# liruiw/OMG-Planner

Measured on AMD Instinct MI355X. Metric: CHOMP iterations/sec (batched scenes) + ms/plan, Panda 7-DoF 30-wp, higher is better.
Workload: dtype f32 SDF / f64 kinematics+update; 1 GPU; 100 table-top scenes/GPU x (64-goal goal-set cost + CHOMP step), Panda 9-dof, 30 waypoints; scenes_per_gpu=100, total_scenes=100, goals=64, waypoints=30, sdf_grid=4x64^3 + 128x96x32 per scene, private, goal_selection=MD on device (omgx_goal_update_optimize), pipeline_parts=3, top_k_collision=1000, plan_restart_every_steps=50

## Files before the change

### omg-planner_amd/csrc/omg_device.h

```cpp
#pragma once
#include <hip/hip_runtime.h>
#include <stdint.h>

#include "../../include/omg_hip.h"

#define OMG_WAVE 64

namespace omg {

struct __attribute__((packed, aligned(4))) F2 { float a, b; };
struct __attribute__((packed, aligned(4))) F4 { float a, b, c, d; };

__device__ __forceinline__ float lerpf(float a, float b, float t) { return __builtin_fmaf(t, b - a, a); }

struct Axis { int i0; float f; bool ok; };
__device__ __forceinline__ Axis axis_of(float g) {
    Axis a;
    a.ok = (g > -1.0e9f) && (g <= 1.0e9f);
    const float s = g - 0.5f;
    a.i0 = (int)s;
    a.f = s - (float)a.i0;
    const bool edge = (s == -1.0f) && (g > -0.5f);
    a.i0 = edge ? 0 : a.i0;
    a.f = edge ? -1.0f : a.f;
// ... 165 lines not shown
        fmx = sdf_value(G, axm, ay, az);
        fmy = sdf_value(G, ax, aym, az);
        fmz = sdf_value(G, ax, ay, azm);
    }
    const float g0 = (float)(0.5 * (double)(fpx - fmx) * o.rdelta);
    const float g1 = (float)(0.5 * (double)(fpy - fmy) * o.rdelta);
    const float g2 = (float)(0.5 * (double)(fpz - fmz) * o.rdelta);
    float v0, v1, v2;
    if (value <= 0.0f) {
        acc.pot += (float)(-(double)value + 0.5 * (double)o.eps);
        v0 = -g0; v1 = -g1; v2 = -g2;
    } else {
        const float d = value - o.eps;
        acc.pot += o.i2eps * d * d * o.pad;
        const float ie = o.ieps;
        v0 = ie * g0 * d * o.pad; v1 = ie * g1 * d * o.pad; v2 = ie * g2 * d * o.pad;
    }
    acc.gx += __builtin_fmaf(T[8], v2, __builtin_fmaf(T[4], v1, T[0] * v0));
    acc.gy += __builtin_fmaf(T[9], v2, __builtin_fmaf(T[5], v1, T[1] * v0));
    acc.gz += __builtin_fmaf(T[10], v2, __builtin_fmaf(T[6], v1, T[2] * v0));
}

template <bool WANT_GRAD>
__device__ __forceinline__ void sdf_pair(const ObjParams& o, const float* __restrict__ grid, float px, float py, float pz,
                                         Accum& acc) {
    const PairPrep pp = pair_prepare(o, px, py, pz);
    if (!pp.far) pair_exact<WANT_GRAD>(o, grid, pp.tx, pp.ty, pp.tz, acc);
}

#define OMG_CONST_AS __attribute__((address_space(4)))
typedef const OMG_CONST_AS omgx_object* ObjTablePtr;
typedef const OMG_CONST_AS int32_t* IntTablePtr;
#define OMG_GLOBAL_AS __attribute__((address_space(1)))
typedef const OMG_GLOBAL_AS char* GlobalBytes;
typedef float F2v __attribute__((ext_vector_type(2), aligned(4)));
__device__ __forceinline__ F2 global_f2(GlobalBytes p) { const F2v v = *(const OMG_GLOBAL_AS F2v*)p; return F2{v.x, v.y}; }
__device__ __forceinline__ ObjTablePtr as_const(const omgx_object* p) { return (ObjTablePtr)(uintptr_t)p; }
__device__ __forceinline__ IntTablePtr as_const(const int32_t* p) { return (IntTablePtr)(uintptr_t)p; }

__device__ __forceinline__ ObjParams load_object(ObjTablePtr ob) {
    ObjParams o;
#pragma unroll
    for (int k = 0; k < 12; ++k) o.T[k] = ob->pose_inv[k];
#pragma unroll
    for (int k = 0; k < 3; ++k) { o.lo[k] = ob->lo[k]; o.hi[k] = ob->hi[k]; o.dim[k] = ob->dim[k]; }
    o.delta = ob->delta; o.eps = ob->epsilon; o.pad = ob->padding_scale; o.clr = ob->clearance;
#pragma unroll
    for (int k = 0; k < 3; ++k) { o.rw[k] = ob->inv_extent[k]; o.rc[k] = ob->rb_c[k]; o.rh[k] = ob->rb_h[k]; }
    o.rr2 = ob->rb_r2;
    o.rdelta = ob->inv_delta; o.i2eps = ob->inv_2eps; o.ieps = ob->inv_eps;
    return o;
}

template <bool WANT_GRAD>
__device__ __forceinline__ Accum sdf_point(const omgx_object* __restrict__ objs, int o_begin, int o_end,
                                           const float* __restrict__ pool, float px, float py, float pz) {
    Accum acc{0.0f, 0.0f, 0.0f, 0.0f, 0.0f};
    for (int o = o_begin; o < o_end; ++o) {
        ObjTablePtr ob = as_const(objs) + o;
        if (ob->disabled > 0) continue;
        const ObjParams op = load_object(ob);
        sdf_pair<WANT_GRAD>(op, pool + ob->grid_offset, px, py, pz, acc);
    }
    return acc;
}

__device__ __forceinline__ void gq_warm_scalar_cache(const omgx_object* objects, int o_begin, int o_end, const double* balls) {
    const omgx_object* ob[8];
#pragma unroll
    for (int k = 0; k < 8; ++k) ob[k] = objects + (o_begin + k < o_end ? o_begin + k : o_end - 1);
#define OMG_WARM_OBJ(N) "s_load_dword s96, %" #N ", 0x0\n\ts_load_dword s97, %" #N ", 0x40\n\ts_load_dword s98, %" #N ", 0x80\n\ts_load_dword s99, %" #N ", 0xb4\n\t"
    asm volatile(OMG_WARM_OBJ(0) OMG_WARM_OBJ(1) OMG_WARM_OBJ(2) OMG_WARM_OBJ(3) OMG_WARM_OBJ(4) OMG_WARM_OBJ(5) OMG_WARM_OBJ(6) OMG_WARM_OBJ(7)
                 "s_load_dword s96, %8, 0x0\n\ts_load_dword s97, %8, 0x40\n\ts_load_dword s98, %8, 0x80\n\ts_load_dword s99, %8, 0xc0\n\t"
                 "s_load_dword s96, %8, 0x100\n\ts_load_dword s97, %8, 0x13c\n\ts_waitcnt lgkmcnt(0)"
                 :
                 : "s"(ob[0]), "s"(ob[1]), "s"(ob[2]), "s"(ob[3]), "s"(ob[4]), "s"(ob[5]), "s"(ob[6]), "s"(ob[7]), "s"(balls)
                 : "s96", "s97", "s98", "s99", "memory");
#undef OMG_WARM_OBJ
}

template <class DPtr>
struct RobotViewT {
    const double* __restrict__ raw;
    DPtr d;
    const double* __restrict__ g;
    int P;
    __device__ __forceinline__ RobotViewT(const double* blob, int P_) : raw(blob), d((DPtr)(uintptr_t)(blob + OMGX_ROBOT_POINTS + 30 * P_)), g(blob + OMGX_ROBOT_POINTS + 30 * P_), P(P_) {}
    __device__ __forceinline__ RobotViewT(const double* blob, int P_, DPtr chain_constants) : raw(blob), d(chain_constants), g(blob + OMGX_ROBOT_POINTS + 30 * P_), P(P_) {}
    __device__ __forceinline__ DPtr uvw(int i) const { return d + 27 * i; }
    __device__ __forceinline__ DPtr tp(int i) const { return d + 189 + 3 * i; }
    __device__ __forceinline__ DPtr hand() const { return d + 210; }
    __device__ __forceinline__ DPtr lf() const { return d + 222; }
    __device__ __forceinline__ DPtr rf() const { return d + 234; }
    __device__ __forceinline__ const double* pts(int l, int p) const { return g + 246 + 3 * (l * P + p); }
    __device__ __forceinline__ DPtr ax(int l) const { return d + 246 + 30 * P + 3 * l; }
    __device__ __forceinline__ DPtr og(int l) const { return d + 276 + 30 * P + 3 * l; }
    __device__ __forceinline__ double radius(int l) const { return d[306 + 30 * P + l]; }
    __device__ __forceinline__ DPtr ball(int l) const { return d + 316 + 30 * P + 4 * l; }
    __device__ __forceinline__ const double* lower() const { return raw + OMGX_ROBOT_LOWER; }
    __device__ __forceinline__ const double* upper() const { return raw + OMGX_ROBOT_UPPER; }
};
typedef RobotViewT<const double*> RobotView;
typedef RobotViewT<const OMG_CONST_AS double*> RobotViewS;

struct Pose { double R[9]; double t[3]; };

// ... 229 lines not shown
```

### omg-planner_amd/csrc/omg_goalset_queue.h

```cpp
#pragma once

#define GQ_TBL_MAX 32
#ifndef GQ_WG_PER_CU
#define GQ_WG_PER_CU 5
#endif
#ifndef GQ_WAVES
#define GQ_WAVES 4
#endif
#define GQ_NT (64 * GQ_WAVES)

struct GqFar {
    float T[12], lo[3], rc[3], rh[3], rr2, rb_r;
    bool cullable;
    int disabled;
};

typedef uint32_t GqU16 __attribute__((ext_vector_type(16)));
typedef uint32_t GqU8 __attribute__((ext_vector_type(8)));
typedef uint32_t GqU4 __attribute__((ext_vector_type(4)));
static_assert(offsetof(omgx_object, pose_inv) == 0 && offsetof(omgx_object, lo) == 0x30 && offsetof(omgx_object, epsilon) == 0x58 &&
              offsetof(omgx_object, clearance) == 0x60 && offsetof(omgx_object, disabled) == 0x64 && offsetof(omgx_object, rb_c) == 0x88 &&
              offsetof(omgx_object, rb_h) == 0x94 && offsetof(omgx_object, rb_r) == 0xa0 && offsetof(omgx_object, rb_r2) == 0xa4 &&
              sizeof(omgx_object) >= 0xa8, "gq_load_far reads the record by byte offsets");
__device__ __forceinline__ GqFar gq_load_far(ObjTablePtr ob) {
    GqU16 a;
    GqU4 b;
    GqU8 c;
    asm volatile("s_load_dwordx16 %0, %3, 0x0\n\ts_load_dwordx4 %1, %3, 0x58\n\ts_load_dwordx8 %2, %3, 0x88\n\ts_waitcnt lgkmcnt(0)"
                 : "=&s"(a), "=&s"(b), "=&s"(c) : "s"((uint64_t)(uintptr_t)ob));
    GqFar f;
#pragma unroll
    for (int k = 0; k < 12; ++k) f.T[k] = __uint_as_float(a[k]);
#pragma unroll
    for (int k = 0; k < 3; ++k) { f.lo[k] = __uint_as_float(a[12 + k]); f.rc[k] = __uint_as_float(c[k]); f.rh[k] = __uint_as_float(c[3 + k]); }
    f.rb_r = __uint_as_float(c[6]);
    f.rr2 = __uint_as_float(c[7]);
    f.cullable = ((int32_t)b[0] < 0x3f800000) & ((int32_t)b[2] <= 0x3f800000);
    f.disabled = (int32_t)b[3];
    return f;
}
__device__ __forceinline__ void se3_apply_s(const float* T, float x, float y, float z, float& ux, float& uy, float& uz) {
    ux = T[3]; uy = T[7]; uz = T[11];
    asm("v_fma_f32 %0, %3, %12, %0\n\tv_fma_f32 %1, %6, %12, %1\n\tv_fma_f32 %2, %9, %12, %2\n\t"
        "v_fma_f32 %0, %4, %13, %0\n\tv_fma_f32 %1, %7, %13, %1\n\tv_fma_f32 %2, %10, %13, %2\n\t"
        "v_fma_f32 %0, %5, %14, %0\n\tv_fma_f32 %1, %8, %14, %1\n\tv_fma_f32 %2, %11, %14, %2"
        : "+v"(ux), "+v"(uy), "+v"(uz)
        : "s"(T[0]), "s"(T[1]), "s"(T[2]), "s"(T[4]), "s"(T[5]), "s"(T[6]), "s"(T[8]), "s"(T[9]), "s"(T[10]), "v"(x), "v"(y), "v"(z));
}
__device__ __forceinline__ unsigned long long wave_ballot(bool b) { return __builtin_amdgcn_ballot_w64(b); }

struct GqLayout {
    int mask_off, tile_off, tbl_off, pts_off, stage_off, fkc_off, objc_off, btab_off, total;
    __host__ __device__ GqLayout(int PS, int MR, int P, int tbl_n, bool with_fkc = false, int waves = GQ_WAVES) {
        mask_off = PS * 90 * 8;
        tile_off = mask_off + 10 * MR * 4;
        tbl_off = mask_off + ((10 * MR * 4 + 16 + 15) & ~15);
        pts_off = tbl_off + tbl_n * 64;
        stage_off = pts_off + ((10 * P * 3 * 8 + 15) & ~15);
        total = stage_off + waves * 64 * 16;
        const int fk = stage_off + PS * 14 * 8 + 16;
        if (total < fk) total = fk;
        total = (total + 15) & ~15;
        fkc_off = total;
        if (with_fkc) total += 246 * 8;
        objc_off = total;
        if (with_fkc) total += 8 * 64 * 5 * 4;
        btab_off = total;
        if (with_fkc) total += PS * 7 * 9 * 8;
    }
};

static inline int gq_choose_tbl_n(int PS, int MR, int P, bool with_fkc = false, int waves = GQ_WAVES) {
    static const int step[] = {26624, 31744, 40960, 53248, 80896, 163840};
    const int base = GqLayout(PS, MR, P, 0, with_fkc, waves).total;
    for (int k = 0; k < 6; ++k)
        if (base + 4 * 64 <= step[k]) {
            const int n = (step[k] - base) / 64;
            return n < GQ_TBL_MAX ? n : GQ_TBL_MAX;
        }
    return 0;
}

struct GqTblRec { double rw[3]; int32_t dim[3]; int64_t goffb; float eps, clr, pad, i2e; };
__device__ __forceinline__ GqTblRec gq_tbl_load(const omgx_object* ob) {
    GqTblRec r;
#pragma unroll
    for (int k = 0; k < 3; ++k) { r.rw[k] = ob->inv_extent[k]; r.dim[k] = ob->dim[k]; }
    r.goffb = ob->grid_offset * 4;
    r.eps = ob->epsilon; r.clr = ob->clearance; r.pad = ob->padding_scale; r.i2e = ob->inv_2eps;
    return r;
}
__device__ __forceinline__ void gq_tbl_store(uint32_t* e, const GqTblRec& r) {
#pragma unroll
    for (int k = 0; k < 3; ++k) {
        e[2 * k] = (uint32_t)__double2loint(r.rw[k]); e[2 * k + 1] = (uint32_t)__double2hiint(r.rw[k]);
        e[6 + k] = (uint32_t)r.dim[k];
    }
    e[9] = (uint32_t)(r.goffb & 0xffffffffll); e[10] = (uint32_t)(r.goffb >> 32);
    e[11] = __float_as_uint(0.5f * r.eps);
    e[12] = __float_as_uint(r.eps); e[13] = __float_as_uint(r.clr);
    e[14] = __float_as_uint(r.pad); e[15] = __float_as_uint(r.i2e);
}
// ... 669 lines not shown
```

### omg-planner_amd/csrc/omg_kernels.hip

```cpp
#include <hip/hip_runtime.h>
#include <hip/hip_ext.h>

#include <stdint.h>
#include <stdio.h>
#include <stdlib.h>
#include <string.h>

#include <mutex>

#include "omg_device.h"
#include "omg_host.h"

using namespace omg;

struct RawObjects {
    const float* __restrict__ pose_init;
    const float* __restrict__ sdf_grids;
    const float* __restrict__ sdf_limits;
    const float* __restrict__ eps;
    const float* __restrict__ pad;
    const float* __restrict__ clr;
    const float* __restrict__ dis;
};

// ... 239 lines not shown
                        if (!__any((many & bit) != 0)) continue;
                        ObjTablePtr ob = as_const(a.objects) + o;
                        if (ob->disabled > 0) continue;
                        const ObjParams op = load_object(ob);
                        const float* grid = a.pool + ob->grid_offset;
                        PairPrep pp[LB];
#pragma unroll
                        for (int k = 0; k < LB; ++k) {
                            pp[k] = pair_prepare(op, px[k], py[k], pz[k]);
                            pp[k].far = pp[k].far || !(msk[k] & bit);
                        }
#pragma unroll
                        for (int k = 0; k < LB; ++k)
                            if (!pp[k].far) pair_exact<WANT_GRAD>(op, grid, pp[k].tx, pp[k].ty, pp[k].tz, acc[k]);
                    }
                }
#pragma unroll
                for (int k = 0; k < LB; ++k) {
                    const int l = l0 + k;
                    if (a.soften && l >= 8) {
                        acc[k].pot *= 0.1f; acc[k].gx *= 0.1f; acc[k].gy *= 0.1f; acc[k].gz *= 0.1f; acc[k].col = 0.0f;
                    }
                    if (a.arc && acc[k].pot != 0.0f) {
                        float qx, qy, qz;
                        pose12_apply(ci > 0 ? base + ((int64_t)l * pstride + ci - 1) * 12 : sbase + (int64_t)l * sstride, rv.pts(l, p), qx, qy, qz);
                        const float vx = (px[k] - qx) * a.inv_dt, vy = (py[k] - qy) * a.inv_dt, vz = (pz[k] - qz) * a.inv_dt;
                        acc[k].pot = acc[k].pot * sqrtf(vx * vx + vy * vy + vz * vz);
                    }
                    const int64_t kk = (out_cfg + l) * P + p;
                    if (a.pot) a.pot[kk] = acc[k].pot;
                    if (a.col) a.col[kk] = acc[k].col;
                    if (WANT_GRAD) { a.grad[3 * kk] = acc[k].gx; a.grad[3 * kk + 1] = acc[k].gy; a.grad[3 * kk + 2] = acc[k].gz; }
                    tsum += acc[k].pot;
                    tcol += acc[k].col;
                }
            }
        }
    }
    if (a.chunk_cost || a.chunk_col) {
        const float ws_ = wave_sum(tsum), wc_ = wave_sum(tcol);
        const int w = threadIdx.x >> 6;
        if ((threadIdx.x & 63) == 0) { red[0][w] = ws_; red[1][w] = wc_; }
        __syncthreads();
        if (threadIdx.x == 0) {
            const int64_t k = (int64_t)s * a.NCH + chunk;
            float c0 = red[0][0], c1 = red[1][0];
#pragma unroll
            for (int w2 = 1; w2 < TPB / 64; ++w2) { c0 += red[0][w2]; c1 += red[1][w2]; }
            if (a.chunk_cost) a.chunk_cost[k] = c0;
            if (a.chunk_col) a.chunk_col[k] = c1;
        }
    }
}
template <bool LAT, bool PERSIST = false>
__device__ __forceinline__ void waypoint_layer_block(const ChunkArgs& a, const int s, const int l_begin, const int l_end,
                                                     const int c_begin, const int c_end, double* lds_pose, uint32_t* rowmask,
                                                     const int o_begin, const int o_end, const RobotViewS& rv, double* fkc,
                                                     const bool warming, float* objc, double* btab) {
    const int n = a.wp_n, P = a.P, PS = a.PS, MR = a.MR;
    const int nloc = c_end - c_begin;
    const double* tr = a.wp_traj + ((int64_t)s * n + c_begin) * 9;
    double* sc = reinterpret_cast<double*>(rowmask);
    auto ldtr = [&](int k) -> double {
        if constexpr (PERSIST) return __hip_atomic_load(tr + k, __ATOMIC_RELAXED, __HIP_MEMORY_SCOPE_AGENT);
        else return tr[k];
    };
    const double fkv = (LAT && threadIdx.x < 246) ? rv.g[threadIdx.x] : 0.0;
    if (warming) gq_warm_scalar_cache(a.objects, o_begin, o_end, a.robot + OMGX_ROBOT_POINTS + 30 * P + 316 + 30 * P);
    for (int t = threadIdx.x; t < nloc * 7; t += 256) {
        const int cfg = t / 7, i = t - cfg * 7;
        double sn, cs;
        fk_joint_sincos(ldtr(cfg * 9 + i), sn, cs);
        sc[2 * t] = sn; sc[2 * t + 1] = cs;
    }
    if (LAT && threadIdx.x < 246) fkc[threadIdx.x] = fkv;
    __syncthreads();
    double* const gpose = (a.wp_pose_out && l_begin == 0) ? a.wp_pose_out + ((int64_t)s * n + c_begin) * 120 : nullptr;
    auto run_chain = [&](const auto& view) {
        for (int t = threadIdx.x; t < nloc * 3; t += 256) {
            const int cfg = t / 3, r = t - cfg * 3;
            fk_chain_row(view, r, sc + 14 * cfg, ldtr(cfg * 9 + 7), ldtr(cfg * 9 + 8), [&](int l, double r0, double r1, double r2, double tt) {
                double* dst = lds_pose + ((size_t)l * PS + cfg) * 9;
                if (r < 2) { dst[3 * r] = r0; dst[3 * r + 1] = r1; dst[3 * r + 2] = r2; }
                dst[6 + r] = tt;
                if (gpose) {
                    double* g = gpose + ((size_t)cfg * 10 + l) * 12;
                    g[3 * r] = r0; g[3 * r + 1] = r1; g[3 * r + 2] = r2; g[9 + r] = tt;
                }
            });
        }
    };
    if constexpr (LAT) {
        const RobotView rvl(a.robot, P, fkc);
        for (int t = threadIdx.x; t < nloc * 7; t += 256) fk_joint_matrix(rvl, t - (t / 7) * 7, sc[2 * t], sc[2 * t + 1], btab + 9 * t);
        __syncthreads();
        for (int t = threadIdx.x; t < nloc * 3; t += 256) {
            const int cfg = t / 3, r = t - cfg * 3;
            fk_chain_row_B(rvl, r, btab + 63 * cfg, ldtr(cfg * 9 + 7), ldtr(cfg * 9 + 8), [&](int l, double r0, double r1, double r2, double tt) {
                double* dst = lds_pose + ((size_t)l * PS + cfg) * 9;
                if (r < 2) { dst[3 * r] = r0; dst[3 * r + 1] = r1; dst[3 * r + 2] = r2; }
                dst[6 + r] = tt;
                if (gpose) {
                    double* g = gpose + ((size_t)cfg * 10 + l) * 12;
                    g[3 * r] = r0; g[3 * r + 1] = r1; g[3 * r + 2] = r2; g[9 + r] = tt;
                }
            });
        }
    } else run_chain(rv);
    __syncthreads();
    for (int row = l_begin * nloc + threadIdx.x; row < l_end * nloc; row += 256) {
        const int l = row / nloc, ci = row - l * nloc;
        const double* A = lds_pose + ((int64_t)l * PS + ci) * 9;
        const auto bl = rv.ball(l);
        float cx, cy, cz;
        link_ball_center(A, A + 3, A + 6, bl, cx, cy, cz);
        const float rad = (float)bl[3] + 1.0e-4f;
        uint32_t m = 0;
        for (int o = o_begin; o < o_end; ++o) {
            ObjTablePtr ob = as_const(a.objects) + o;
            if (ob->disabled > 0) continue;
            const int oo = o - o_begin;
            const uint32_t bit = 1u << (oo < 31 ? oo : 31);
            const float ux = __builtin_fmaf(ob->pose_inv[2], cz, __builtin_fmaf(ob->pose_inv[1], cy, __builtin_fmaf(ob->pose_inv[0], cx, ob->pose_inv[3]))) - ob->lo[0];
            const float uy = __builtin_fmaf(ob->pose_inv[6], cz, __builtin_fmaf(ob->pose_inv[5], cy, __builtin_fmaf(ob->pose_inv[4], cx, ob->pose_inv[7]))) - ob->lo[1];
            const float uz = __builtin_fmaf(ob->pose_inv[10], cz, __builtin_fmaf(ob->pose_inv[9], cy, __builtin_fmaf(ob->pose_inv[8], cx, ob->pose_inv[11]))) - ob->lo[2];
            const float rbc[3] = {ob->rb_c[0], ob->rb_c[1], ob->rb_c[2]}, rbh[3] = {ob->rb_h[0], ob->rb_h[1], ob->rb_h[2]};
            const bool near = rbox_near(ux, uy, uz, rad, rbc, rbh, ob->rb_r);
            const bool cullable = ob->epsilon < 1.0f && ob->clearance <= 1.0f;
            if (near || !cullable) m |= bit;
        }
        rowmask[l * MR + ci] = m;
    }
    __syncthreads();
    if (LAT && nloc <= 4 && l_end - l_begin == 1) {
        const int l = l_begin, lane = threadIdx.x & 63, wave = threadIdx.x >> 6;
        const int p = lane & 15, ci = lane >> 4;
        const bool valid = (p < P) && (ci < nloc);
        const int cic = valid ? ci : 0, pc = valid ? p : 0;
        const uint32_t msk = valid ? rowmask[l * MR + cic] : 0u;
        Accum acc{0.0f, 0.0f, 0.0f, 0.0f, 0.0f};
        if (__any(msk != 0)) {
            float px, py, pz;
            pose9_apply(lds_pose + ((int64_t)l * PS + cic) * 9, rv.pts(l, pc), px, py, pz);
            for (int og = o_begin; og < o_end; og += 8) {
                for (int o = og + wave; o < og + 8 && o < o_end; o += 4) {
                    const int oo = o - o_begin;
                    const uint32_t bit = 1u << (oo < 31 ? oo : 31);
                    Accum c{0.0f, 0.0f, 0.0f, 0.0f, 0.0f};
                    if (__any((msk & bit) != 0)) {
                        ObjTablePtr ob = as_const(a.objects) + o;
                        if (!(ob->disabled > 0)) {
                            const ObjParams op = load_object(ob);
                            const PairPrep pp = pair_prepare(op, px, py, pz);
                            if ((msk & bit) && !pp.far) pair_exact<true>(op, a.pool + ob->grid_offset, pp.tx, pp.ty, pp.tz, c);
                        }
                    }
                    float* dst = objc + ((o - og) * 64 + lane) * 5;
                    dst[0] = c.pot; dst[1] = c.gx; dst[2] = c.gy; dst[3] = c.gz; dst[4] = c.col;
                }
                __syncthreads();
                if (wave == 0) {
                    for (int o = og; o < og + 8 && o < o_end; ++o) {
                        const float* src = objc + ((o - og) * 64 + lane) * 5;
                        acc.pot += src[0]; acc.gx += src[1]; acc.gy += src[2]; acc.gz += src[3]; acc.col += src[4];
                    }
                }
                __syncthreads();
            }
        }
        if (wave == 0) {
            if (a.wp_soften && l >= 8) {
                acc.pot *= 0.1f; acc.gx *= 0.1f; acc.gy *= 0.1f; acc.gz *= 0.1f; acc.col = 0.0f;
            }
            if (valid) {
                const int64_t kk = (((int64_t)s * n + c_begin + ci) * 10 + l) * P + p;
                a.wp_pot[kk] = acc.pot;
                a.wp_col[kk] = acc.col;
                a.wp_grad[3 * kk] = acc.gx; a.wp_grad[3 * kk + 1] = acc.gy; a.wp_grad[3 * kk + 2] = acc.gz;
            }
        }
        return;
    }
    const int p = threadIdx.x & 15, r = threadIdx.x >> 4;
    for (int ci0 = 0; ci0 < nloc; ci0 += 16) {
        const int ci = ci0 + r;
        const bool valid = (p < P) && (ci < nloc);
        const int cic = valid ? ci : 0, pc = valid ? p : 0;
#pragma unroll 1
        for (int l = l_begin; l < l_end; ++l) {
            const uint32_t msk = valid ? rowmask[l * MR + cic] : 0u;
            Accum acc{0.0f, 0.0f, 0.0f, 0.0f, 0.0f};
            if (__any(msk != 0)) {
                float px, py, pz;
                pose9_apply(lds_pose + ((int64_t)l * PS + cic) * 9, rv.pts(l, pc), px, py, pz);
                for (int o = o_begin; o < o_end; ++o) {
                    const int oo = o - o_begin;
                    const uint32_t bit = 1u << (oo < 31 ? oo : 31);
                    if (!__any((msk & bit) != 0)) continue;
                    ObjTablePtr ob = as_const(a.objects) + o;
                    if (ob->disabled > 0) continue;
                    const ObjParams op = load_object(ob);
                    const PairPrep pp = pair_prepare(op, px, py, pz);
                    if ((msk & bit) && !pp.far) pair_exact<true>(op, a.pool + ob->grid_offset, pp.tx, pp.ty, pp.tz, acc);
                }
            }
            if (a.wp_soften && l >= 8) {
                acc.pot *= 0.1f; acc.gx *= 0.1f; acc.gy *= 0.1f; acc.gz *= 0.1f; acc.col = 0.0f;
            }
            if (valid) {
                const int64_t kk = (((int64_t)s * n + c_begin + ci) * 10 + l) * P + p;
                a.wp_pot[kk] = acc.pot;
                a.wp_col[kk] = acc.col;
                a.wp_grad[3 * kk] = acc.gx; a.wp_grad[3 * kk + 1] = acc.gy; a.wp_grad[3 * kk + 2] = acc.gz;
            }
        }
    }
}

#ifdef OMGX_GS_CLOCK
__device__ unsigned long long g_gs_wg[1 << 16][8];
#define GS_WG_IDX ((blockIdx.x + (((unsigned)a.S & 1u) << 14)) & 0xffffu)
#define GS_WG_STAMP(k) do { if (threadIdx.x == 0 && blockIdx.x < (1u << 16)) { g_gs_wg[GS_WG_IDX][k] = wall_clock64(); if (k == 0) { g_gs_wg[GS_WG_IDX][5] = ~0ull; g_gs_wg[GS_WG_IDX][6] = 0ull; unsigned hw, xcc; asm volatile("s_getreg_b32 %0, hwreg(HW_REG_HW_ID)" : "=s"(hw)); asm volatile("s_getreg_b32 %0, hwreg(HW_REG_XCC_ID)" : "=s"(xcc)); g_gs_wg[GS_WG_IDX][7] = ((unsigned long long)xcc << 32) | hw; } } } while (0)
__device__ unsigned long long g_gs_wave[1 << 16][8];
#define GS_WAVE_STAMP(k) do { if ((threadIdx.x & 63) == 0 && (k) < 8 && blockIdx.x < (1u << 16)) g_gs_wave[blockIdx.x][k] = wall_clock64(); } while (0)
extern "C" int omgx_debug_gs_wave(unsigned long long* h_out, int n_wg) {
    if (n_wg > (1 << 16)) n_wg = 1 << 16;
    return hipMemcpyFromSymbol(h_out, HIP_SYMBOL(g_gs_wave), sizeof(unsigned long long) * 8 * n_wg) == hipSuccess ? 0 : -2;
}
__device__ unsigned long long g_gs_freq[1 << 16][2];
#define GS_FREQ_BEGIN() unsigned long long gs_f0 = 0, gs_f1 = 0; if (threadIdx.x == 0) { gs_f0 = __builtin_readcyclecounter(); gs_f1 = wall_clock64(); }
#define GS_FREQ_END() do { if (threadIdx.x == 0 && blockIdx.x < (1u << 16)) { g_gs_freq[blockIdx.x][0] = __builtin_readcyclecounter() - gs_f0; g_gs_freq[blockIdx.x][1] = wall_clock64() - gs_f1; } } while (0)
extern "C" int omgx_debug_gs_freq(unsigned long long* h_out, int n_wg) {
    if (n_wg > (1 << 16)) n_wg = 1 << 16;
    return hipMemcpyFromSymbol(h_out, HIP_SYMBOL(g_gs_freq), sizeof(unsigned long long) * 2 * n_wg) == hipSuccess ? 0 : -2;
}
extern "C" int omgx_debug_gs_wg(unsigned long long* h_out, int n_wg) {
    if (n_wg > (1 << 16)) n_wg = 1 << 16;
    return hipMemcpyFromSymbol(h_out, HIP_SYMBOL(g_gs_wg), sizeof(unsigned long long) * 8 * n_wg) == hipSuccess ? 0 : -2;
}
#else
#define GS_WG_STAMP(k)
#define GS_WAVE_STAMP(k)
#define GS_FREQ_BEGIN()
#define GS_FREQ_END()
#endif

#if defined(OMGX_GS_ADD_S)
#define GS_MARGINAL_COST_PROBE(a_, b_, c_, d_, i_, j_) do { { uint32_t d0 = (uint32_t)(i_), d1 = (uint32_t)(j_); asm volatile("s_add_u32 %0, %0, 3\n\ts_add_u32 %1, %1, 5\n\ts_add_u32 %0, %0, 3\n\ts_add_u32 %1, %1, 5\n\ts_add_u32 %0, %0, 3\n\ts_add_u32 %1, %1, 5\n\ts_add_u32 %0, %0, 3\n\ts_add_u32 %1, %1, 5\n\t" "s_add_u32 %0, %0, 3\n\ts_add_u32 %1, %1, 5\n\ts_add_u32 %0, %0, 3\n\ts_add_u32 %1, %1, 5\n\ts_add_u32 %0, %0, 3\n\ts_add_u32 %1, %1, 5\n\ts_add_u32 %0, %0, 3\n\ts_add_u32 %1, %1, 5" : "+s"(d0), "+s"(d1) : : "scc"); } } while (0)
#elif defined(OMGX_GS_ADD_V)
#define GS_MARGINAL_COST_PROBE(a_, b_, c_, d_, i_, j_) do { { float d0 = (a_), d1 = (b_), d2 = (c_), d3 = (d_); asm volatile("v_fma_f32 %0, %0, %0, %0\n\tv_fma_f32 %1, %1, %1, %1\n\tv_fma_f32 %2, %2, %2, %2\n\tv_fma_f32 %3, %3, %3, %3\n\t" "v_fma_f32 %0, %0, %0, %0\n\tv_fma_f32 %1, %1, %1, %1\n\tv_fma_f32 %2, %2, %2, %2\n\tv_fma_f32 %3, %3, %3, %3\n\t" "v_fma_f32 %0, %0, %0, %0\n\tv_fma_f32 %1, %1, %1, %1\n\tv_fma_f32 %2, %2, %2, %2\n\tv_fma_f32 %3, %3, %3, %3\n\t" "v_fma_f32 %0, %0, %0, %0\n\tv_fma_f32 %1, %1, %1, %1\n\tv_fma_f32 %2, %2, %2, %2\n\tv_fma_f32 %3, %3, %3, %3" : "+v"(d0), "+v"(d1), "+v"(d2), "+v"(d3)); } } while (0)
#elif defined(OMGX_GS_ADD_V64)
#define GS_MARGINAL_COST_PROBE(a_, b_, c_, d_, i_, j_) do { { double d0 = (a_), d1 = (b_), d2 = (c_), d3 = (d_); asm volatile("v_fma_f64 %0, %0, %0, %0\n\tv_fma_f64 %1, %1, %1, %1\n\tv_fma_f64 %2, %2, %2, %2\n\tv_fma_f64 %3, %3, %3, %3\n\t" "v_fma_f64 %0, %0, %0, %0\n\tv_fma_f64 %1, %1, %1, %1\n\tv_fma_f64 %2, %2, %2, %2\n\tv_fma_f64 %3, %3, %3, %3\n\t" "v_fma_f64 %0, %0, %0, %0\n\tv_fma_f64 %1, %1, %1, %1\n\tv_fma_f64 %2, %2, %2, %2\n\tv_fma_f64 %3, %3, %3, %3\n\t" "v_fma_f64 %0, %0, %0, %0\n\tv_fma_f64 %1, %1, %1, %1\n\tv_fma_f64 %2, %2, %2, %2\n\tv_fma_f64 %3, %3, %3, %3" : "+v"(d0), "+v"(d1), "+v"(d2), "+v"(d3)); } } while (0)
#elif defined(OMGX_GS_ADD_B)
#define GS_MARGINAL_COST_PROBE(a_, b_, c_, d_, i_, j_) do { asm volatile("s_branch 1f\n\ts_nop 0\n\t1:\n\ts_branch 2f\n\ts_nop 0\n\t2:\n\ts_branch 3f\n\ts_nop 0\n\t3:\n\ts_branch 4f\n\ts_nop 0\n\t4:\n\t" "s_branch 5f\n\ts_nop 0\n\t5:\n\ts_branch 6f\n\ts_nop 0\n\t6:\n\ts_branch 7f\n\ts_nop 0\n\t7:\n\ts_branch 8f\n\ts_nop 0\n\t8:"); } while (0)
#elif defined(OMGX_GS_ADD_N)
#define GS_MARGINAL_COST_PROBE(a_, b_, c_, d_, i_, j_) do { asm volatile("s_nop 0\n\ts_nop 0\n\ts_nop 0\n\ts_nop 0\n\ts_nop 0\n\ts_nop 0\n\ts_nop 0\n\ts_nop 0\n\ts_nop 0\n\ts_nop 0\n\ts_nop 0\n\ts_nop 0\n\ts_nop 0\n\ts_nop 0\n\ts_nop 0\n\ts_nop 0"); } while (0)
#else
#define GS_MARGINAL_COST_PROBE(a_, b_, c_, d_, i_, j_) do { } while (0)
#endif

#ifdef OMGX_GS_COUNT
__device__ unsigned long long g_gs_count[16];
#define GS_COUNT(k) do { if ((threadIdx.x & 63) == 0) atomicAdd(&g_gs_count[k], 1ull); } while (0)
#define GS_COUNT_N(k, n) do { const unsigned long long n_ = (unsigned long long)(n); if ((threadIdx.x & 63) == 0) atomicAdd(&g_gs_count[k], n_); } while (0)
extern "C" int omgx_debug_gs_counts(unsigned long long* h_out, int reset) {
    if (hipMemcpyFromSymbol(h_out, HIP_SYMBOL(g_gs_count), sizeof(unsigned long long) * 16) != hipSuccess) return -2;
    if (reset) { unsigned long long z[16] = {}; if (hipMemcpyToSymbol(HIP_SYMBOL(g_gs_count), z, sizeof(z)) != hipSuccess) return -2; }
    return 0;
}
#else
#define GS_COUNT(k)
#define GS_COUNT_N(k, n)
#endif


#include "omg_goalset_kin.h"
#include "omg_goalset_queue.h"

static thread_local char g_err[256] = "";

int omgx_set_error(const char* what, hipError_t e) {
    snprintf(g_err, sizeof g_err, "%s: %s", what, hipGetErrorString(e));
    return OMGX_ERR_LAUNCH;
}
extern "C" const char* omgx_last_error(void) { return g_err; }

#define OMGX_TIMING_CAP 4096
static std::mutex g_timing_mu;
static bool g_timing = false;
static int g_timing_dev = -1;
static int g_timing_stride = 1, g_timing_seen = 0;
static int g_timing_n = 0;
static hipEvent_t g_ev[OMGX_TIMING_CAP][2];
static bool g_ev_made[OMGX_TIMING_CAP];
static int g_ev_kind[OMGX_TIMING_CAP];

extern "C" int omgx_timing_enable(int32_t on) {
    std::lock_guard<std::mutex> lock(g_timing_mu);
// ... 902 lines not shown
```

Measured before the change: 552,000 iterations/s.

## Software-pipeline SDF pair gathers across objects in waypoint layer block

Rewrites the per-waypoint object loop in waypoint_layer_block so the grid gathers for the next live object are issued before the current object's trilinear and gradient math is consumed. This hides global-load latency behind arithmetic. It also switches the broad-phase mask pass to batched scalar record loads and scalar-operand SE3 transforms, and replaces the per-object __any checks with a wave-uniform OR of the row masks. In exchange it uses more registers for the in-flight gather state, which could lower occupancy. The lambda-based prefetch also adds control-flow complexity.

```diff
diff --git a/omg-planner_amd/csrc/omg_device.h b/omg-planner_amd/csrc/omg_device.h
--- a/omg-planner_amd/csrc/omg_device.h
+++ b/omg-planner_amd/csrc/omg_device.h
@@ -241,6 +241,182 @@
     return o;
 }
 
+struct GqFar {
+    float T[12], lo[3], rc[3], rh[3], rr2, rb_r;
+    bool cullable;
+    int disabled;
+};
+
+typedef uint32_t GqU16 __attribute__((ext_vector_type(16)));
+typedef uint32_t GqU8 __attribute__((ext_vector_type(8)));
+typedef uint32_t GqU4 __attribute__((ext_vector_type(4)));
+static_assert(offsetof(omgx_object, pose_inv) == 0 && offsetof(omgx_object, lo) == 0x30 && offsetof(omgx_object, epsilon) == 0x58 &&
+              offsetof(omgx_object, clearance) == 0x60 && offsetof(omgx_object, disabled) == 0x64 && offsetof(omgx_object, rb_c) == 0x88 &&
+              offsetof(omgx_object, rb_h) == 0x94 && offsetof(omgx_object, rb_r) == 0xa0 && offsetof(omgx_object, rb_r2) == 0xa4 &&
+              sizeof(omgx_object) >= 0xa8, "gq_load_far reads the record by byte offsets");
+__device__ __forceinline__ GqFar gq_load_far(ObjTablePtr ob) {
+    GqU16 a;
+    GqU4 b;
+    GqU8 c;
+    asm volatile("s_load_dwordx16 %0, %3, 0x0\n\ts_load_dwordx4 %1, %3, 0x58\n\ts_load_dwordx8 %2, %3, 0x88\n\ts_waitcnt lgkmcnt(0)"
+                 : "=&s"(a), "=&s"(b), "=&s"(c) : "s"((uint64_t)(uintptr_t)ob));
+    GqFar f;
+#pragma unroll
+    for (int k = 0; k < 12; ++k) f.T[k] = __uint_as_float(a[k]);
+#pragma unroll
+    for (int k = 0; k < 3; ++k) { f.lo[k] = __uint_as_float(a[12 + k]); f.rc[k] = __uint_as_float(c[k]); f.rh[k] = __uint_as_float(c[3 + k]); }
+    f.rb_r = __uint_as_float(c[6]);
+    f.rr2 = __uint_as_float(c[7]);
+    f.cullable = ((int32_t)b[0] < 0x3f800000) & ((int32_t)b[2] <= 0x3f800000);
+    f.disabled = (int32_t)b[3];
+    return f;
+}
+__device__ __forceinline__ void se3_apply_s(const float* T, float x, float y, float z, float& ux, float& uy, float& uz) {
+    ux = T[3]; uy = T[7]; uz = T[11];
+    asm("v_fma_f32 %0, %3, %12, %0\n\tv_fma_f32 %1, %6, %12, %1\n\tv_fma_f32 %2, %9, %12, %2\n\t"
+        "v_fma_f32 %0, %4, %13, %0\n\tv_fma_f32 %1, %7, %13, %1\n\tv_fma_f32 %2, %10, %13, %2\n\t"
+        "v_fma_f32 %0, %5, %14, %0\n\tv_fma_f32 %1, %8, %14, %1\n\tv_fma_f32 %2, %11, %14, %2"
+        : "+v"(ux), "+v"(uy), "+v"(uz)
+        : "s"(T[0]), "s"(T[1]), "s"(T[2]), "s"(T[4]), "s"(T[5]), "s"(T[6]), "s"(T[8]), "s"(T[9]), "s"(T[10]), "v"(x), "v"(y), "v"(z));
+}
+__device__ __forceinline__ unsigned long long wave_ballot(bool b) { return __builtin_amdgcn_ballot_w64(b); }
+
+
+struct GqPairRec {
+    GqFar f;
+    int dim[3];
+    int64_t grid_offset;
+    double rw[3];
+};
+static_assert(offsetof(omgx_object, dim) == 0x48 && offsetof(omgx_object, grid_offset) == 0x68 && offsetof(omgx_object, inv_extent) == 0x70,
+              "gq_load_pair reads the record by byte offsets");
+__device__ __forceinline__ GqPairRec gq_load_pair(ObjTablePtr ob) {
+    GqU16 a, b;
+    GqU8 c;
+    asm volatile("s_load_dwordx16 %0, %3, 0x0\n\ts_load_dwordx16 %1, %3, 0x48\n\ts_load_dwordx8 %2, %3, 0x88\n\ts_waitcnt lgkmcnt(0)"
+                 : "=&s"(a), "=&s"(b), "=&s"(c) : "s"((uint64_t)(uintptr_t)ob));
+    GqPairRec r;
+#pragma unroll
+    for (int k = 0; k < 12; ++k) r.f.T[k] = __uint_as_float(a[k]);
+#pragma unroll
+    for (int k = 0; k < 3; ++k) {
+        r.f.lo[k] = __uint_as_float(a[12 + k]); r.f.rc[k] = __uint_as_float(c[k]); r.f.rh[k] = __uint_as_float(c[3 + k]);
+        r.dim[k] = (int)b[k];
+        r.rw[k] = __hiloint2double((int)b[11 + 2 * k], (int)b[10 + 2 * k]);
+    }
+    r.f.rb_r = __uint_as_float(c[6]);
+    r.f.rr2 = __uint_as_float(c[7]);
+    r.f.cullable = ((int32_t)b[4] < 0x3f800000) & ((int32_t)b[6] <= 0x3f800000);
+    r.f.disabled = (int32_t)b[7];
+    r.grid_offset = (int64_t)(((uint64_t)b[9] << 32) | (uint64_t)b[8]);
+    return r;
+}
+
+typedef float F4v __attribute__((ext_vector_type(4), aligned(4)));
+__device__ __forceinline__ F4 global_f4(GlobalBytes p) { const F4v v = *(const OMG_GLOBAL_AS F4v*)p; return F4{v.x, v.y, v.z, v.w}; }
+struct PairGathers {
+    F4 c00, c01, c10, c11;
+    F2 xp0, xp1, xm0, xm1, yp0, yp1, ym0, ym1;
+    float gx, gy, gz;
+};
+__device__ __forceinline__ unsigned long long pair_exact_issue(const double* rw, const int* dim, const float* grid, float tx, float ty, float tz,
+                                                               bool live, PairGathers& g) {
+    const float gx = (float)((double)tx * rw[0]) * (float)dim[0];
+    const float gy = (float)((double)ty * rw[1]) * (float)dim[1];
+    const float gz = (float)((double)tz * rw[2]) * (float)dim[2];
+    const int dx = dim[0], dy = dim[1], dz = dim[2];
+    const Axis ax = axis_of(gx), ay = axis_of(gy), az = axis_of(gz);
+    const bool in_c = ax.ok && ay.ok && az.ok && ax.i0 >= 0 && ax.i0 < dx - 1 && ay.i0 >= 0 && ay.i0 < dy - 1 && az.i0 >= 0 && az.i0 < dz - 1;
+    const Axis axp = axis_of(gx + 1.0f), axm = axis_of(gx - 1.0f);
+    const Axis ayp = axis_of(gy + 1.0f), aym = axis_of(gy - 1.0f);
+    const Axis azp = axis_of(gz + 1.0f), azm = axis_of(gz - 1.0f);
+    const bool regular = axp.i0 == ax.i0 + 1 && axm.i0 == ax.i0 - 1 && ayp.i0 == ay.i0 + 1 && aym.i0 == ay.i0 - 1 &&
+                         azp.i0 == az.i0 + 1 && azm.i0 == az.i0 - 1 && axp.ok && axm.ok && ayp.ok && aym.ok && azp.ok && azm.ok;
+    const bool interior = in_c && regular && ax.i0 >= 1 && ax.i0 < dx - 2 && ay.i0 >= 1 && ay.i0 < dy - 2 && az.i0 >= 1 && az.i0 < dz - 2;
+    const bool take = live && interior;
+    const uint32_t b = take ? (uint32_t)((ax.i0 * dy + ay.i0) * dz + az.i0) * 4u : 4u;
+    const uint32_t sy = take ? (uint32_t)dz * 4u : 0u, sx = take ? (uint32_t)(dy * dz) * 4u : 0u;
+    const GlobalBytes c = (GlobalBytes)(uintptr_t)grid;
+    g.c00 = global_f4(c + (b - 4u));
+    g.c01 = global_f4(c + (b + sy - 4u));
+    g.c10 = global_f4(c + (b + sx - 4u));
+    g.c11 = global_f4(c + (b + sx + sy - 4u));
+    g.xp0 = global_f2(c + (b + 2u * sx));
+    g.xp1 = global_f2(c + (b + 2u * sx + sy));
+    g.xm0 = global_f2(c + (b - sx));
+    g.xm1 = global_f2(c + (b - sx + sy));
+    g.yp0 = global_f2(c + (b + 2u * sy));
+    g.yp1 = global_f2(c + (b + sx + 2u * sy));
+    g.ym0 = global_f2(c + (b - sy));
+    g.ym1 = global_f2(c + (b + sx - sy));
+    g.gx = gx; g.gy = gy; g.gz = gz;
+    return wave_ballot(take);
+}
+__device__ __forceinline__ void pair_exact_consume(const ObjParams& o, const float* __restrict__ grid, const PairGathers& g, bool interior,
+                                                   Accum& acc) {
+    const float* T = o.T;
+    const float gx = g.gx, gy = g.gy, gz = g.gz;
+    Grid G{grid, o.dim[0], o.dim[1], o.dim[2]};
+    const Axis ax = axis_of(gx), ay = axis_of(gy), az = axis_of(gz);
+    const Axis axp = axis_of(gx + 1.0f), axm = axis_of(gx - 1.0f);
+    const Axis ayp = axis_of(gy + 1.0f), aym = axis_of(gy - 1.0f);
+    const Axis azp = axis_of(gz + 1.0f), azm = axis_of(gz - 1.0f);
+    bool in_c = true;
+    if (!interior) {
+        in_c = ax.ok && ay.ok && az.ok && ax.i0 >= 0 && ax.i0 < G.dx - 1 && ay.i0 >= 0 && ay.i0 < G.dy - 1 && az.i0 >= 0 && az.i0 < G.dz - 1;
+        if (!in_c) {
+            if (1.0f < o.clr) acc.col += 1.0f;
+            if (!(1.0f <= o.eps)) return;
+        }
+    }
+
+    float value, fpx, fmx, fpy, fmy, fpz, fmz;
+    if (interior) {
+        const F4 &c00 = g.c00, &c01 = g.c01, &c10 = g.c10, &c11 = g.c11;
+        value = trilerp(c00.b, c00.c, c01.b, c01.c, c10.b, c10.c, c11.b, c11.c, ax.f, ay.f, az.f);
+        if (value < o.clr) acc.col += 1.0f;
+        if (!(value <= 0.0f || value <= o.eps)) return;
+        fpz = trilerp(c00.c, c00.d, c01.c, c01.d, c10.c, c10.d, c11.c, c11.d, ax.f, ay.f, azp.f);
+        fmz = trilerp(c00.a, c00.b, c01.a, c01.b, c10.a, c10.b, c11.a, c11.b, ax.f, ay.f, azm.f);
+        fpx = trilerp(c10.b, c10.c, c11.b, c11.c, g.xp0.a, g.xp0.b, g.xp1.a, g.xp1.b, axp.f, ay.f, az.f);
+        fmx = trilerp(g.xm0.a, g.xm0.b, g.xm1.a, g.xm1.b, c00.b, c00.c, c01.b, c01.c, axm.f, ay.f, az.f);
+        fpy = trilerp(c01.b, c01.c, g.yp0.a, g.yp0.b, c11.b, c11.c, g.yp1.a, g.yp1.b, ax.f, ayp.f, az.f);
+        fmy = trilerp(g.ym0.a, g.ym0.b, c00.b, c00.c, g.ym1.a, g.ym1.b, c10.b, c10.c, ax.f, aym.f, az.f);
+    } else {
+        Grid Gs = G;
+        asm volatile("" : "+s"(Gs.dy), "+s"(Gs.dz));
+        if (in_c) {
+            value = sdf_value(Gs, ax, ay, az);
+            if (value < o.clr) acc.col += 1.0f;
+            if (!(value <= 0.0f || value <= o.eps)) return;
+        } else {
+            value = 1.0f;
+        }
+        fpx = sdf_value(Gs, axp, ay, az);
+        fpy = sdf_value(Gs, ax, ayp, az);
+        fpz = sdf_value(Gs, ax, ay, azp);
+        fmx = sdf_value(Gs, axm, ay, az);
+        fmy = sdf_value(Gs, ax, aym, az);
+        fmz = sdf_value(Gs, ax, ay, azm);
+    }
+    const float g0 = (float)(0.5 * (double)(fpx - fmx) * o.rdelta);
+    const float g1 = (float)(0.5 * (double)(fpy - fmy) * o.rdelta);
+    const float g2 = (float)(0.5 * (double)(fpz - fmz) * o.rdelta);
+    float v0, v1, v2;
+    if (value <= 0.0f) {
+        acc.pot += (float)(-(double)value + 0.5 * (double)o.eps);
+        v0 = -g0; v1 = -g1; v2 = -g2;
+    } else {
+        const float d = value - o.eps;
+        acc.pot += o.i2eps * d * d * o.pad;
+        const float ie = o.ieps;
+        v0 = ie * g0 * d * o.pad; v1 = ie * g1 * d * o.pad; v2 = ie * g2 * d * o.pad;
+    }
+    acc.gx += __builtin_fmaf(T[8], v2, __builtin_fmaf(T[4], v1, T[0] * v0));
+    acc.gy += __builtin_fmaf(T[9], v2, __builtin_fmaf(T[5], v1, T[1] * v0));
+    acc.gz += __builtin_fmaf(T[10], v2, __builtin_fmaf(T[6], v1, T[2] * v0));
+}
+
 template <bool WANT_GRAD>
 __device__ __forceinline__ Accum sdf_point(const omgx_object* __restrict__ objs, int o_begin, int o_end,
                                            const float* __restrict__ pool, float px, float py, float pz) {
diff --git a/omg-planner_amd/csrc/omg_goalset_queue.h b/omg-planner_amd/csrc/omg_goalset_queue.h
--- a/omg-planner_amd/csrc/omg_goalset_queue.h
+++ b/omg-planner_amd/csrc/omg_goalset_queue.h
@@ -8,46 +8,6 @@
 #define GQ_WAVES 4
 #endif
 #define GQ_NT (64 * GQ_WAVES)
-
-struct GqFar {
-    float T[12], lo[3], rc[3], rh[3], rr2, rb_r;
-    bool cullable;
-    int disabled;
-};
-
-typedef uint32_t GqU16 __attribute__((ext_vector_type(16)));
-typedef uint32_t GqU8 __attribute__((ext_vector_type(8)));
-typedef uint32_t GqU4 __attribute__((ext_vector_type(4)));
-static_assert(offsetof(omgx_object, pose_inv) == 0 && offsetof(omgx_object, lo) == 0x30 && offsetof(omgx_object, epsilon) == 0x58 &&
-              offsetof(omgx_object, clearance) == 0x60 && offsetof(omgx_object, disabled) == 0x64 && offsetof(omgx_object, rb_c) == 0x88 &&
-              offsetof(omgx_object, rb_h) == 0x94 && offsetof(omgx_object, rb_r) == 0xa0 && offsetof(omgx_object, rb_r2) == 0xa4 &&
-              sizeof(omgx_object) >= 0xa8, "gq_load_far reads the record by byte offsets");
-__device__ __forceinline__ GqFar gq_load_far(ObjTablePtr ob) {
-    GqU16 a;
-    GqU4 b;
-    GqU8 c;
-    asm volatile("s_load_dwordx16 %0, %3, 0x0\n\ts_load_dwordx4 %1, %3, 0x58\n\ts_load_dwordx8 %2, %3, 0x88\n\ts_waitcnt lgkmcnt(0)"
-                 : "=&s"(a), "=&s"(b), "=&s"(c) : "s"((uint64_t)(uintptr_t)ob));
-    GqFar f;
-#pragma unroll
-    for (int k = 0; k < 12; ++k) f.T[k] = __uint_as_float(a[k]);
-#pragma unroll
-    for (int k = 0; k < 3; ++k) { f.lo[k] = __uint_as_float(a[12 + k]); f.rc[k] = __uint_as_float(c[k]); f.rh[k] = __uint_as_float(c[3 + k]); }
-    f.rb_r = __uint_as_float(c[6]);
-    f.rr2 = __uint_as_float(c[7]);
-    f.cullable = ((int32_t)b[0] < 0x3f800000) & ((int32_t)b[2] <= 0x3f800000);
-    f.disabled = (int32_t)b[3];
-    return f;
-}
-__device__ __forceinline__ void se3_apply_s(const float* T, float x, float y, float z, float& ux, float& uy, float& uz) {
-    ux = T[3]; uy = T[7]; uz = T[11];
-    asm("v_fma_f32 %0, %3, %12, %0\n\tv_fma_f32 %1, %6, %12, %1\n\tv_fma_f32 %2, %9, %12, %2\n\t"
-        "v_fma_f32 %0, %4, %13, %0\n\tv_fma_f32 %1, %7, %13, %1\n\tv_fma_f32 %2, %10, %13, %2\n\t"
-        "v_fma_f32 %0, %5, %14, %0\n\tv_fma_f32 %1, %8, %14, %1\n\tv_fma_f32 %2, %11, %14, %2"
-        : "+v"(ux), "+v"(uy), "+v"(uz)
-        : "s"(T[0]), "s"(T[1]), "s"(T[2]), "s"(T[4]), "s"(T[5]), "s"(T[6]), "s"(T[8]), "s"(T[9]), "s"(T[10]), "v"(x), "v"(y), "v"(z));
-}
-__device__ __forceinline__ unsigned long long wave_ballot(bool b) { return __builtin_amdgcn_ballot_w64(b); }
 
 struct GqLayout {
     int mask_off, tile_off, tbl_off, pts_off, stage_off, fkc_off, objc_off, btab_off, total;
diff --git a/omg-planner_amd/csrc/omg_kernels.hip b/omg-planner_amd/csrc/omg_kernels.hip
--- a/omg-planner_amd/csrc/omg_kernels.hip
+++ b/omg-planner_amd/csrc/omg_kernels.hip
@@ -315,6 +315,34 @@
         }
     }
 }
+#ifdef OMGX_GS_CLOCK
+__device__ unsigned long long g_gs_wg[1 << 16][8];
+#define GS_WG_IDX ((blockIdx.x + (((unsigned)a.S & 1u) << 14)) & 0xffffu)
+#define GS_WG_STAMP(k) do { if (threadIdx.x == 0 && blockIdx.x < (1u << 16)) { g_gs_wg[GS_WG_IDX][k] = wall_clock64(); if (k == 0) { g_gs_wg[GS_WG_IDX][5] = ~0ull; g_gs_wg[GS_WG_IDX][6] = 0ull; unsigned hw, xcc; asm volatile("s_getreg_b32 %0, hwreg(HW_REG_HW_ID)" : "=s"(hw)); asm volatile("s_getreg_b32 %0, hwreg(HW_REG_XCC_ID)" : "=s"(xcc)); g_gs_wg[GS_WG_IDX][7] = ((unsigned long long)xcc << 32) | hw; } } } while (0)
+__device__ unsigned long long g_gs_wave[1 << 16][8];
+#define GS_WAVE_STAMP(k) do { if ((threadIdx.x & 63) == 0 && (k) < 8 && blockIdx.x < (1u << 16)) g_gs_wave[blockIdx.x][k] = wall_clock64(); } while (0)
+extern "C" int omgx_debug_gs_wave(unsigned long long* h_out, int n_wg) {
+    if (n_wg > (1 << 16)) n_wg = 1 << 16;
+    return hipMemcpyFromSymbol(h_out, HIP_SYMBOL(g_gs_wave), sizeof(unsigned long long) * 8 * n_wg) == hipSuccess ? 0 : -2;
+}
+__device__ unsigned long long g_gs_freq[1 << 16][2];
+#define GS_FREQ_BEGIN() unsigned long long gs_f0 = 0, gs_f1 = 0; if (threadIdx.x == 0) { gs_f0 = __builtin_readcyclecounter(); gs_f1 = wall_clock64(); }
+#define GS_FREQ_END() do { if (threadIdx.x == 0 && blockIdx.x < (1u << 16)) { g_gs_freq[blockIdx.x][0] = __builtin_readcyclecounter() - gs_f0; g_gs_freq[blockIdx.x][1] = wall_clock64() - gs_f1; } } while (0)
+extern "C" int omgx_debug_gs_freq(unsigned long long* h_out, int n_wg) {
+    if (n_wg > (1 << 16)) n_wg = 1 << 16;
+    return hipMemcpyFromSymbol(h_out, HIP_SYMBOL(g_gs_freq), sizeof(unsigned long long) * 2 * n_wg) == hipSuccess ? 0 : -2;
+}
+extern "C" int omgx_debug_gs_wg(unsigned long long* h_out, int n_wg) {
+    if (n_wg > (1 << 16)) n_wg = 1 << 16;
+    return hipMemcpyFromSymbol(h_out, HIP_SYMBOL(g_gs_wg), sizeof(unsigned long long) * 8 * n_wg) == hipSuccess ? 0 : -2;
+}
+#else
+#define GS_WG_STAMP(k)
+#define GS_WAVE_STAMP(k)
+#define GS_FREQ_BEGIN()
+#define GS_FREQ_END()
+#endif
+
 template <bool LAT, bool PERSIST = false>
 __device__ __forceinline__ void waypoint_layer_block(const ChunkArgs& a, const int s, const int l_begin, const int l_end,
                                                      const int c_begin, const int c_end, double* lds_pose, uint32_t* rowmask,
@@ -371,6 +399,7 @@
         }
     } else run_chain(rv);
     __syncthreads();
+    GS_WG_STAMP(2);
     for (int row = l_begin * nloc + threadIdx.x; row < l_end * nloc; row += 256) {
         const int l = row / nloc, ci = row - l * nloc;
         const double* A = lds_pose + ((int64_t)l * PS + ci) * 9;
@@ -380,21 +409,19 @@
         const float rad = (float)bl[3] + 1.0e-4f;
         uint32_t m = 0;
         for (int o = o_begin; o < o_end; ++o) {
-            ObjTablePtr ob = as_const(a.objects) + o;
-            if (ob->disabled > 0) continue;
+            const GqFar f = gq_load_far(as_const(a.objects) + o);
+            if (f.disabled > 0) continue;
             const int oo = o - o_begin;
             const uint32_t bit = 1u << (oo < 31 ? oo : 31);
-            const float ux = __builtin_fmaf(ob->pose_inv[2], cz, __builtin_fmaf(ob->pose_inv[1], cy, __builtin_fmaf(ob->pose_inv[0], cx, ob->pose_inv[3]))) - ob->lo[0];
-            const float uy = __builtin_fmaf(ob->pose_inv[6], cz, __builtin_fmaf(ob->pose_inv[5], cy, __builtin_fmaf(ob->pose_inv[4], cx, ob->pose_inv[7]))) - ob->lo[1];
-            const float uz = __builtin_fmaf(ob->pose_inv[10], cz, __builtin_fmaf(ob->pose_inv[9], cy, __builtin_fmaf(ob->pose_inv[8], cx, ob->pose_inv[11]))) - ob->lo[2];
-            const float rbc[3] = {ob->rb_c[0], ob->rb_c[1], ob->rb_c[2]}, rbh[3] = {ob->rb_h[0], ob->rb_h[1], ob->rb_h[2]};
-            const bool near = rbox_near(ux, uy, uz, rad, rbc, rbh, ob->rb_r);
-            const bool cullable = ob->epsilon < 1.0f && ob->clearance <= 1.0f;
-            if (near || !cullable) m |= bit;
+            float ux, uy, uz;
+            se3_apply_s(f.T, cx, cy, cz, ux, uy, uz);
+            const bool near = rbox_near(ux - f.lo[0], uy - f.lo[1], uz - f.lo[2], rad, f.rc, f.rh, f.rb_r);
+            if (near || !f.cullable) m |= bit;
         }
         rowmask[l * MR + ci] = m;
     }
     __syncthreads();
+    GS_WG_STAMP(3);
     if (LAT && nloc <= 4 && l_end - l_begin == 1) {
         const int l = l_begin, lane = threadIdx.x & 63, wave = threadIdx.x >> 6;
         const int p = lane & 15, ci = lane >> 4;
@@ -452,19 +479,52 @@
 #pragma unroll 1
         for (int l = l_begin; l < l_end; ++l) {
             const uint32_t msk = valid ? rowmask[l * MR + cic] : 0u;
+            const uint32_t sm = (uint32_t)__builtin_amdgcn_readlane((int)msk, 0) | (uint32_t)__builtin_amdgcn_readlane((int)msk, 16) |
+                                (uint32_t)__builtin_amdgcn_readlane((int)msk, 32) | (uint32_t)__builtin_amdgcn_readlane((int)msk, 48);
             Accum acc{0.0f, 0.0f, 0.0f, 0.0f, 0.0f};
-            if (__any(msk != 0)) {
+            if (sm != 0) {
                 float px, py, pz;
                 pose9_apply(lds_pose + ((int64_t)l * PS + cic) * 9, rv.pts(l, pc), px, py, pz);
-                for (int o = o_begin; o < o_end; ++o) {
-                    const int oo = o - o_begin;
-                    const uint32_t bit = 1u << (oo < 31 ? oo : 31);
-                    if (!__any((msk & bit) != 0)) continue;
-                    ObjTablePtr ob = as_const(a.objects) + o;
-                    if (ob->disabled > 0) continue;
+                int o = o_begin;
+                double rw[3] = {0.0, 0.0, 0.0};
+                int dim[3] = {0, 0, 0};
+                const float* grid = a.pool;
+                float tx = 0.0f, ty = 0.0f, tz = 0.0f;
+                unsigned long long live_mask = 0;
+                int o_of = o_begin;
+                auto prepare = [&]() -> bool {
+                    while (o < o_end) {
+                        const int oc = o++;
+                        const int oo = oc - o_begin, sh = oo < 31 ? oo : 31;
+                        if (!((sm >> sh) & 1u)) continue;
+                        const GqPairRec rec = gq_load_pair(as_const(a.objects) + oc);
+                        if (rec.f.disabled > 0) continue;
+                        float ux, uy, uz;
+                        se3_apply_s(rec.f.T, px, py, pz, ux, uy, uz);
+                        const float sx_ = ux - rec.f.lo[0], sy_ = uy - rec.f.lo[1], sz_ = uz - rec.f.lo[2];
+                        const bool reach = ((msk >> sh) & 1u) != 0, inside = rbox_inside(sx_, sy_, sz_, rec.f.rc, rec.f.rh, rec.f.rr2);
+                        const unsigned long long lm = wave_ballot(reach) & (wave_ballot(inside) | (rec.f.cullable ? 0ull : ~0ull));
+                        if (lm == 0) continue;
+                        tx = sx_; ty = sy_; tz = sz_;
+                        live_mask = lm;
+                        o_of = oc;
+#pragma unroll
+                        for (int k = 0; k < 3; ++k) { rw[k] = rec.rw[k]; dim[k] = rec.dim[k]; }
+                        grid = a.pool + rec.grid_offset;
+                        return true;
+                    }
+                    return false;
+                };
+                bool more = prepare();
+                while (more) {
+                    PairGathers g;
+                    const unsigned long long in_mask = pair_exact_issue(rw, dim, grid, tx, ty, tz, __builtin_amdgcn_inverse_ballot_w64(live_mask), g);
+                    const unsigned long long cur_mask = live_mask;
+                    ObjTablePtr ob = as_const(a.objects) + o_of;
+                    const float* const cur_grid = grid;
+                    more = prepare();
                     const ObjParams op = load_object(ob);
-                    const PairPrep pp = pair_prepare(op, px, py, pz);
-                    if ((msk & bit) && !pp.far) pair_exact<true>(op, a.pool + ob->grid_offset, pp.tx, pp.ty, pp.tz, acc);
+                    if (__builtin_amdgcn_inverse_ballot_w64(cur_mask)) pair_exact_consume(op, cur_grid, g, __builtin_amdgcn_inverse_ballot_w64(in_mask), acc);
                 }
             }
             if (a.wp_soften && l >= 8) {
@@ -479,34 +539,6 @@
         }
     }
 }
-
-#ifdef OMGX_GS_CLOCK
-__device__ unsigned long long g_gs_wg[1 << 16][8];
-#define GS_WG_IDX ((blockIdx.x + (((unsigned)a.S & 1u) << 14)) & 0xffffu)
-#define GS_WG_STAMP(k) do { if (threadIdx.x == 0 && blockIdx.x < (1u << 16)) { g_gs_wg[GS_WG_IDX][k] = wall_clock64(); if (k == 0) { g_gs_wg[GS_WG_IDX][5] = ~0ull; g_gs_wg[GS_WG_IDX][6] = 0ull; unsigned hw, xcc; asm volatile("s_getreg_b32 %0, hwreg(HW_REG_HW_ID)" : "=s"(hw)); asm volatile("s_getreg_b32 %0, hwreg(HW_REG_XCC_ID)" : "=s"(xcc)); g_gs_wg[GS_WG_IDX][7] = ((unsigned long long)xcc << 32) | hw; } } } while (0)
-__device__ unsigned long long g_gs_wave[1 << 16][8];
-#define GS_WAVE_STAMP(k) do { if ((threadIdx.x & 63) == 0 && (k) < 8 && blockIdx.x < (1u << 16)) g_gs_wave[blockIdx.x][k] = wall_clock64(); } while (0)
-extern "C" int omgx_debug_gs_wave(unsigned long long* h_out, int n_wg) {
-    if (n_wg > (1 << 16)) n_wg = 1 << 16;
-    return hipMemcpyFromSymbol(h_out, HIP_SYMBOL(g_gs_wave), sizeof(unsigned long long) * 8 * n_wg) == hipSuccess ? 0 : -2;
-}
-__device__ unsigned long long g_gs_freq[1 << 16][2];
-#define GS_FREQ_BEGIN() unsigned long long gs_f0 = 0, gs_f1 = 0; if (threadIdx.x == 0) { gs_f0 = __builtin_readcyclecounter(); gs_f1 = wall_clock64(); }
-#define GS_FREQ_END() do { if (threadIdx.x == 0 && blockIdx.x < (1u << 16)) { g_gs_freq[blockIdx.x][0] = __builtin_readcyclecounter() - gs_f0; g_gs_freq[blockIdx.x][1] = wall_clock64() - gs_f1; } } while (0)
-extern "C" int omgx_debug_gs_freq(unsigned long long* h_out, int n_wg) {
-    if (n_wg > (1 << 16)) n_wg = 1 << 16;
-    return hipMemcpyFromSymbol(h_out, HIP_SYMBOL(g_gs_freq), sizeof(unsigned long long) * 2 * n_wg) == hipSuccess ? 0 : -2;
-}
-extern "C" int omgx_debug_gs_wg(unsigned long long* h_out, int n_wg) {
-    if (n_wg > (1 << 16)) n_wg = 1 << 16;
-    return hipMemcpyFromSymbol(h_out, HIP_SYMBOL(g_gs_wg), sizeof(unsigned long long) * 8 * n_wg) == hipSuccess ? 0 : -2;
-}
-#else
-#define GS_WG_STAMP(k)
-#define GS_WAVE_STAMP(k)
-#define GS_FREQ_BEGIN()
-#define GS_FREQ_END()
-#endif
 
 #if defined(OMGX_GS_ADD_S)
 #define GS_MARGINAL_COST_PROBE(a_, b_, c_, d_, i_, j_) do { { uint32_t d0 = (uint32_t)(i_), d1 = (uint32_t)(j_); asm volatile("s_add_u32 %0, %0, 3\n\ts_add_u32 %1, %1, 5\n\ts_add_u32 %0, %0, 3\n\ts_add_u32 %1, %1, 5\n\ts_add_u32 %0, %0, 3\n\ts_add_u32 %1, %1, 5\n\ts_add_u32 %0, %0, 3\n\ts_add_u32 %1, %1, 5\n\t" "s_add_u32 %0, %0, 3\n\ts_add_u32 %1, %1, 5\n\ts_add_u32 %0, %0, 3\n\ts_add_u32 %1, %1, 5\n\ts_add_u32 %0, %0, 3\n\ts_add_u32 %1, %1, 5\n\ts_add_u32 %0, %0, 3\n\ts_add_u32 %1, %1, 5" : "+s"(d0), "+s"(d1) : : "scc"); } } while (0)
```

Measured after the change: 550,400 iterations/s. Within noise of the previous version (-0.3%).
